# carsonswope/3d-beats

Hardware: AMD Instinct MI355X
Metric: classified Mpix/s on 848x480 depth frames (4 trees, depth 20); % of the bounding roofline level (roofline.bound; HBM: roofline.hbm_frac) (higher is better)
Workload: dtype f32

## Files before the change

3d-beats_amd/csrc/rdf_hip.hip:

```cpp

#include <hip/hip_runtime.h>
#include <stdint.h>
#include <stdio.h>
#include <stdlib.h>
#include <string.h>
#include <time.h>
#include <unistd.h>

#include <algorithm>
#include <array>
#include <atomic>
#include <mutex>
#include <utility>
#include <vector>

#include "../../include/rdf_hip.h"
#include "rdf_device.hpp"
#include "rdf_host_state.hpp"
#include "rdf_launch_plan.hpp"

namespace {

constexpr uint32_t kFlagLeftLeaf = 1u, kFlagRightLeaf = 2u, kFlagExact = 4u;
using rdf_host::kSchedSlots;
// ... 446 lines not shown
                    }
                }
            } else {
                const float *pp = a.forest +
                    ((size_t)tree * (size_t)a.nodes + (leaf >> 1)) * (size_t)a.E +
                    7 + (leaf & 1u) * a.C + c0;
#pragma unroll
                for (int c = 0; c < CMAX; c += 4) {
                    if (c0 + c + 3 < a.C) {
                        const f4u v = *reinterpret_cast<const f4u *>(pp + c);
                        pdf[c] = pdf[c] + v.x; pdf[c + 1] = pdf[c + 1] + v.y;
                        pdf[c + 2] = pdf[c + 2] + v.z; pdf[c + 3] = pdf[c + 3] + v.w;
                    } else {
#pragma unroll
                        for (int e = 0; e < 4; ++e)
                            if (c0 + c + e < a.C) pdf[c + e] = pdf[c + e] + pp[c + e];
                    }
                }
            }
            return true;
        };
        uint32_t tw_h = kIdle, tw_i = 0u;
        bool tw_valid = false;
        for (uint32_t first = TW ? (tw_row < tile_rows ? tw_row * 64u : n_valid) : wave * 64u; first < n_valid; first += BLOCK) {
            const uint32_t slot = first + (uint32_t)lane;
            uint32_t entry = slot;
            bool live = true;
            if (compact) {
                if (slot >= n_valid) {
                    if (!DEEP) continue;
                    live = false;
                }
                entry = px_list[live ? slot : first];
            }
            const int ly = (int)(y0 + (entry >> 6) * fold + ((entry & 63u) >> col_shift));
            const int px = (int)(x0 + (entry & ((1u << col_shift) - 1u)));
            if (!compact && (ly >= a.Hl || px >= a.Wl)) {
                if (!DEEP) continue;
                live = false;
            }
            const uint32_t i = img_loff + (uint32_t)ly * (uint32_t)a.Wl + (uint32_t)px;
            const int x = px * a.r, y = ly * a.r;
            const int xl = x - tx0, yl = y - ty0;
            bool skip = false;
            if (!compact && live && a.filter_class != -1) skip = (int)a.filter[i] != a.filter_class;
            uint32_t d = 0u;
            if (!skip && live) d = (uint32_t)tprobe_value(tprobe_issue(pc, (uint32_t)xl * 2u, (uint32_t)yl));
            if (!compact && live && (skip || d == 0u || d == kNoPixel)) {
                if (a.fill_untouched && (!TW || tw_tree == 0u)) a.labels[i] = (uint16_t)kNoPixel;
                if (!DEEP) continue;
                live = false;
            }
            if (DEEP && !live) d = 1u;
            const float df = (float)d;
            const float r0 = __builtin_amdgcn_rcpf(df);
            const float rcp = __builtin_fmaf(__builtin_fmaf(-df, r0, 1.0f), r0, r0);
            float rcp_s = rcp * (1.0f / kNumScale);
            const float df_s = df * kNumScale;
            uint32_t kx2 = ((uint32_t)xl - kMagicBits) * 2u;
            const uint32_t ky = (uint32_t)yl - kMagicBits;
            pin(kx2);

            float best = 0.0f;
            int best_c = 0;
            bool any_leaf = false;

            for (int c0 = 0; c0 < a.C || c0 == 0; c0 += CMAX) {
                float pdf[CMAX];
#pragma unroll
                for (int c = 0; c < CMAX; ++c) pdf[c] = 0.0f;

                for (int kb = TW ? (int)tw_tree : 0; kb < (TW ? (int)tw_tree + 1 : a.T); kb += GROUP) {
                    uint32_t h[GROUP];
#pragma unroll
                    for (int k = 0; k < GROUP; ++k) h[k] = (live && (kb + k) < a.T) ? 1u : kIdle;

#pragma unroll
                    for (int c = 0; c < CMAX; ++c) pin(pdf[c]);
                    const bool fast_levels = PACKED || K > 0;
                    if (fast_levels) set_round_down(rcp_s);

                    int j = 0;
                    if constexpr (kPlainLevels) {
                        if (a.plain_levels != 0 && kb + GROUP <= a.T && !__any(!live)) {
                            for (; j < walk_levels; ++j) {
                                Node n[GROUP];
                                if (j < K) {
#pragma unroll
                                    for (int k = 0; k < GROUP; ++k) {
                                        const uint32_t tk = (uint32_t)min(kb + k, a.T - 1);
                                        n[k] = decode_node(lds_nodes[tk * lds_pitch + h[k]]);
                                    }
                                } else {
#pragma unroll
                                    for (int k = 0; k < GROUP; ++k) {
                                        const int tk = min(kb + k, a.T - 1);
                                        const char *base = reinterpret_cast<const char *>(a.packed16 + ((size_t)tk << a.D));
                                        n[k] = decode_node(*reinterpret_cast<const uint4 *>(base + h[k] * 16u));
                                    }
                                }
                                uint32_t fl = 0u;
#pragma unroll
                                for (int k = 0; k < GROUP; ++k) fl |= n[k].flags;
                                if (__any((fl & (kFlagLeftLeaf | kFlagRightLeaf | kFlagExact)) != 0u)) break;
                                TileProbe qu[GROUP], qv[GROUP];
#pragma unroll
                                for (int k = 0; k < GROUP; ++k) {
                                    const f2 nu = {n[k].ax, n[k].ay};
                                    const f2 nv = {n[k].bx, n[k].by};
                                    const f2 r2 = {rcp_s, rcp_s};
                                    const f2 m2 = {kMagic, kMagic};
                                    const f2 tu = __builtin_elementwise_fma(nu, r2, m2);
                                    const f2 tv = __builtin_elementwise_fma(nv, r2, m2);
                                    qu[k] = tprobe_issue(pc, (__float_as_uint(tu.x) << 1) + kx2, __float_as_uint(tu.y) + ky);
                                    qv[k] = tprobe_issue(pc, (__float_as_uint(tv.x) << 1) + kx2, __float_as_uint(tv.y) + ky);
                                }
#pragma unroll
                                for (int k = 0; k < GROUP; ++k) {
                                    const int g = tprobe_value(qu[k]) - tprobe_value(qv[k]) - (int)n[k].lo16;
                                    h[k] = walk_step_plain(h[k], g, n[k].w2);
                                }
                            }
                        }
                    }

                    for (; j < walk_levels; ++j) {
                        bool any = false;
#pragma unroll
                        for (int k = 0; k < GROUP; ++k) any |= (int)h[k] > 0;
                        if (!__any(any)) break;

                        const bool in_lds = j < K;
                        float df_e = df;
                        if (!PACKED && fast_levels && j == K) set_round_nearest(df_e);
                        Node n[GROUP];
                        uint32_t hn[GROUP];
#pragma unroll
                        for (int k = 0; k < GROUP; ++k) hn[k] = (uint32_t)max((int)h[k], (PACKED || in_lds) ? 0 : 1 << j);
                        if (in_lds) {
#pragma unroll
                            for (int k = 0; k < GROUP; ++k) {
                                const uint32_t tk = (uint32_t)min(kb + k, a.T - 1);
                                n[k] = decode_node(lds_nodes[tk * lds_pitch + hn[k]]);
                                if (STATS && c0 == 0) st_lds += (int)h[k] > 0 ? 1u : 0u;
                            }
                        } else if (PACKED) {
#pragma unroll
                            for (int k = 0; k < GROUP; ++k) {
                                const int tk = min(kb + k, a.T - 1);
                                const char *base = reinterpret_cast<const char *>(a.packed16 + ((size_t)tk << a.D));
                                n[k] = decode_node(*reinterpret_cast<const uint4 *>(base + hn[k] * 16u));
                                if (STATS && c0 == 0) st_rec += lines_of((int)h[k] > 0, hn[k] * 16u);
                            }
                        } else {
#pragma unroll
                            for (int k = 0; k < GROUP; ++k) {
                                const int tk = min(kb + k, a.T - 1);
                                const float *p = a.forest + ((size_t)tk * (size_t)a.nodes + (hn[k] - 1u)) * (size_t)a.E;
                                if (STATS && c0 == 0) st_rec += lines_of((int)h[k] > 0, (hn[k] - 1u) * (uint32_t)a.E * 4u);
                                const f4u uv = *reinterpret_cast<const f4u *>(p);
                                const f3u tf = *reinterpret_cast<const f3u *>(p + 4);
                                n[k].ax = a.s * uv.x; n[k].ay = a.s * uv.y; n[k].bx = a.s * uv.z; n[k].by = a.s * uv.w;
                                set_threshold(n[k], thresh_to_int(tf.x));
                                n[k].flags = child_flags(tf.y, tf.z) | kFlagExact;
                            }
                        }

                        uint32_t ux[GROUP], uy[GROUP], vx[GROUP], vy[GROUP];
                        uint32_t fl = 0u;
#pragma unroll
                        for (int k = 0; k < GROUP; ++k) fl |= n[k].flags;
                        if (__any((fl & kFlagExact) != 0u)) {
                            const bool switch_mode = PACKED || in_lds;
                            if (switch_mode) set_round_nearest(df_e);
                            if (PACKED || in_lds) {
#pragma unroll
                                for (int k = 0; k < GROUP; ++k) {
                                    if (n[k].flags & kFlagExact) {
                                        const int tk = min(kb + k, a.T - 1);
                                        if (a.forest) {
                                            const float s_exact = (PACKED && a.info) ? a.info->scale : a.s;
                                            const float *p = a.forest +
                                                ((size_t)tk * (size_t)a.nodes + (hn[k] - 1u)) * (size_t)a.E;
                                            n[k].ax = s_exact * p[0]; n[k].ay = s_exact * p[1];
                                            n[k].bx = s_exact * p[2]; n[k].by = s_exact * p[3];
                                        } else {
                                            n[k].ax = n[k].ay = n[k].bx = n[k].by = 0.0f;
                                            if (a.stale_flag) __hip_atomic_store(a.stale_flag, 1u, __ATOMIC_RELAXED, __HIP_MEMORY_SCOPE_SYSTEM);
                                        }
                                    }
                                }
                            }
#pragma unroll
                            for (int k = 0; k < GROUP; ++k) {
                                const float den = (n[k].flags & kFlagExact) ? df_e : df_s;
                                ux[k] = (uint32_t)min(max(add_wrap(xl, floor_i32(n[k].ax / den)), -(1 << 30)), (1 << 30) - 1) * 2u;
                                uy[k] = (uint32_t)add_wrap(yl, floor_i32(n[k].ay / den));
                                vx[k] = (uint32_t)min(max(add_wrap(xl, floor_i32(n[k].bx / den)), -(1 << 30)), (1 << 30) - 1) * 2u;
                                vy[k] = (uint32_t)add_wrap(yl, floor_i32(n[k].by / den));
                            }
                            if (switch_mode) {
#pragma unroll
                                for (int k = 0; k < GROUP; ++k) { pin(ux[k]); pin(uy[k]); pin(vx[k]); pin(vy[k]); }
                                set_round_down(ux[0]);
// ... 274 lines not shown
                int best_c = 0;
                bool any_leaf = false;
                for (int c0 = 0; c0 < a.C || c0 == 0; c0 += CMAX) {
                    float pdf[CMAX];
#pragma unroll
                    for (int c = 0; c < CMAX; ++c) pdf[c] = 0.0f;
                    for (uint32_t t = 0; t < tw_T; ++t)
                        any_leaf |= add_leaf_pdf(xch[(tw_row * tw_T + t) * 64u + (uint32_t)lane], (int)t, c0, pdf);
#pragma unroll
                    for (int c = 0; c < CMAX; ++c) {
                        if (c0 + c < a.C && pdf[c] > best) {
                            best = pdf[c];
                            best_c = c0 + c;
                        }
                    }
                }
                if (a.keep_if_no_leaf && !any_leaf) {
                    if (a.fill_untouched) a.labels[tw_i] = (uint16_t)kNoPixel;
                } else {
                    a.labels[tw_i] = (uint16_t)best_c;
                }
            }
        }
        if (!TW && more_tiles) {
            uint32_t before = 0u;
            if (lane == 0) before = atomicAdd(&s_tile[4u + (it & 1u)], 1u);
            scout = __builtin_amdgcn_readfirstlane((int)before) == 0;
        }
    }

    if (PACKED && a.info && a.stale_flag && block_id == n_blocks - 1u && tid == 0 && !a.q_helper) {
        if (a.info->generation != a.expect_gen)
            __hip_atomic_store(a.stale_flag, 1u, __ATOMIC_RELAXED, __HIP_MEMORY_SCOPE_SYSTEM);
    }

    if (a.sched && queued != 0u && tid == 0) {
        const unsigned int done = atomicAdd(a.sched + 8 * kSchedStride, 1u);
        if (done == q_blocks - 1u) {
            for (int q = 0; q < 9; ++q) atomicExch(a.sched + q * kSchedStride, 0u);
        }
    }

    if (STATS) {
        uint32_t c[8] = {st_px, st_lv, st_lf, st_lds, st_rec, st_leaf, st_far, st_blk};
#pragma unroll
        for (int i = 0; i < 8; ++i) {
            unsigned long long v = c[i];
            for (int o = 32; o > 0; o >>= 1) v += __shfl_down(v, o);
            if (lane == 0 && (i < 3 || a.stats_wide)) atomicAdd(a.stats + i, v);
        }
    }
}

__global__ __launch_bounds__(256) void k_pack(const float *forest, NodeRec16 *packed16, PackInfo *info,
                                              float *packed_pdf, LastLevelRec *last_level, unsigned int *last_level_unusable,
                                              uint4 *deep, int n_trees, int C, int cpad,
                                              size_t total_slots, int D, int E, float s, int force_exact, uint32_t generation)
{
    const size_t slot = (size_t)blockIdx.x * 256 + threadIdx.x;
    if (slot >= total_slots) return;
    const size_t tree = slot >> D, h = slot & (((size_t)1 << D) - 1);
    if (h == 0) {
        NodeRec16 z16 = {{0u, 0u, 0u, 0u}};
        packed16[slot] = z16;
        for (int c = 0; c < 2 * cpad; ++c) packed_pdf[slot * 2 * (size_t)cpad + c] = 0.f;
        if (tree == 0) {
            info->scale = s; info->magic = kPackMagic; info->generation = generation;
            info->n_trees = (uint32_t)n_trees; info->max_depth = (uint32_t)D; info->n_classes = (uint32_t)C;
        }
        if (deep && tree == 0) {
            uint4 *z = deep + (deep_total_lines(n_trees, D, cpad) << 3);
            for (int i = 0; i < 8; ++i) z[i] = make_uint4(0u, 0u, 0u, 0u);
        }
        return;
    }
    const size_t i = tree * ((((size_t)1) << D) - 1) + (h - 1);
    const float *p = forest + i * (size_t)E;
    struct { uint32_t flags; } n;
    NodeRec16 h16 = encode_node(s * p[0], s * p[1], s * p[2], s * p[3], p[4], p[5], p[6]);
    if (force_exact) h16.w[3] |= kFlagExact;
    n.flags = h16.w[3] & 0xFFu;
    packed16[slot] = h16;
    if (n.flags & kFlagExact) atomicAdd(&info->exact_nodes, 1u);
    float *q = packed_pdf + slot * 2 * (size_t)cpad;
    for (int c = 0; c < cpad; ++c) {
        q[c] = c < C ? p[7 + c] : 0.f;
        q[cpad + c] = c < C ? p[7 + C + c] : 0.f;
    }
    if (deep) {
        const int R0 = D - deep_last_levels(cpad), Lmin = R0 % 3;
        const int j = 63 - __clzll((unsigned long long)h);
        if (j >= Lmin) {
            const int R = j >= R0 ? R0 : R0 - 3 * ((R0 - j + 2) / 3);
            const int t = j - R;
            const size_t line = deep_lines_before(n_trees, R, Lmin) + (tree << R) + ((h >> t) - ((size_t)1 << R));
            uint4 *blk = deep + (line << 3);
            const uint4 rec = make_uint4(h16.w[0], h16.w[1], h16.w[2], h16.w[3]);
            const float4 *pq = reinterpret_cast<const float4 *>(q);
            const uint4 z = make_uint4(0u, 0u, 0u, 0u);
            if (R == R0 && cpad == 8) {
                blk[0] = rec; blk[1] = z; blk[6] = z; blk[7] = z;
                for (int i = 0; i < 4; ++i) reinterpret_cast<float4 *>(blk)[2 + i] = pq[i];
            } else {
                blk[((1u << t) - 1u) + (uint32_t)(h & ((1u << t) - 1u))] = rec;
                if (t == 0) blk[7] = z;
                if (R == R0 && t == 1) {
                    const uint32_t c = (uint32_t)(h & 1u);
                    reinterpret_cast<float4 *>(blk)[3 + 2 * c] = pq[0];
                    reinterpret_cast<float4 *>(blk)[4 + 2 * c] = pq[1];
                }
            }
            unsigned int *tr = reinterpret_cast<unsigned int *>(deep + ((deep_total_lines(n_trees, D, cpad) + 1u) << 3));
            if (n.flags & kFlagExact) atomicMax(tr, (unsigned)j + 1u);
            if (j == D - 1 && (n.flags & 7u) != (kFlagLeftLeaf | kFlagRightLeaf)) atomicAdd(tr + 1, 1u);
        }
    }
    const size_t first = (size_t)1 << (D - 1);
    if (last_level && h >= first) {
        LastLevelRec r;
        r.node = h16;
        for (int c = 0; c < 4; ++c) {
            r.pdf_left[c] = q[c];
            r.pdf_right[c] = q[4 + c];
            r.pad[c] = 0u;
        }
        last_level[(tree << (D - 1)) + (h - first)] = r;
        const bool unusable = (n.flags & 7u) != (kFlagLeftLeaf | kFlagRightLeaf);
        const float *pp = forest + (tree * ((((size_t)1) << D) - 1) + ((h >> 1) - 1)) * (size_t)E;
        const float to_me = pp[5 + (h & 1)];
        const bool in_use = to_me >= -1.0f && to_me < 0.0f;
        const unsigned long long bu = __ballot(unusable), bi = __ballot(in_use);
        const unsigned long long mine = __ballot(true);
        if ((unsigned)__lane_id() == (unsigned)__ffsll((long long)mine) - 1u) {
            if (bu) atomicAdd(last_level_unusable, (unsigned)__popcll(bu));
            if (bi) atomicAdd(last_level_unusable + 1, (unsigned)__popcll(bi));
        }
    }
}

constexpr int kMaxSpecLayers = 4;
struct SpecFilters {
    int n;
    int fl[kMaxSpecLayers], fc[kMaxSpecLayers];
};

__global__ __launch_bounds__(256) void k_composite(const uint16_t *const *imgs, int n_images, uint32_t n_px,
                                                   const int2 *cond, int n_cond, uint16_t *out, int32_t *bad,
                                                   int fill_untouched, uint32_t flip_w, const uint32_t *colors,
                                                   int num_colors, uint32_t *rgba, const SpecFilters spec)
{
    const uint32_t p = blockIdx.x * 256u + threadIdx.x;
    if (p >= n_px) return;
    uint32_t lab[kMaxSpecLayers];
    if (spec.n > 0) {
#pragma unroll
        for (int i = 0; i < kMaxSpecLayers; ++i) {
            lab[i] = kNoPixel;
            if (i < spec.n) {
                uint32_t l = imgs[i][p];
                if (spec.fl[i] >= 0) {
                    uint32_t f = kNoPixel;
#pragma unroll
                    for (int j = 0; j < kMaxSpecLayers; ++j)
                        if (j < i && j == spec.fl[i]) f = lab[j];
                    if ((int)f != spec.fc[i] && l != kNoPixel) {
                        l = kNoPixel;
// ... 226 lines not shown
            *split->launched = (int)hgrid;
            return (int)hipGetLastError();
        }
    }
    hipLaunchKernelGGL(kern, dim3((unsigned)grid), dim3(block), lds_bytes, st, ka);
    return (int)hipGetLastError();
}

template <int NL>
int launch_multi(ForestKernel<NL> kern, int block, const EvalArgsN<NL> &ka, int lds_bytes, DeviceState &ds, int cus, hipStream_t st)
{
    int per_cu = 0;
    const int rc = workgroups_per_cu(ds, reinterpret_cast<const void *>(kern), block, lds_bytes, &per_cu);
    if (rc != RDF_OK) return rc;
    long long per_role = (long long)cus * per_cu / NL;
    uint32_t most_tiles = 0;
    for (int l = 0; l < NL; ++l) most_tiles = ka.l[l].n_tiles > most_tiles ? ka.l[l].n_tiles : most_tiles;
    if (per_role > (long long)most_tiles) per_role = most_tiles;
    if (per_role < 1) per_role = 1;
    hipLaunchKernelGGL(kern, dim3((unsigned)(per_role * NL)), dim3(block), lds_bytes, st, ka);
    return (int)hipGetLastError();
}

StaleFlag make_stale_flag()
{
    StaleFlag f;
    void *h = nullptr, *d = nullptr;
    if (hipHostMalloc(&h, 64, hipHostMallocMapped) == hipSuccess && h) {
        memset(h, 0, 64);
        if (hipHostGetDevicePointer(&d, h, 0) == hipSuccess && d) {
            f.host = reinterpret_cast<unsigned int *>(h);
            f.dev = reinterpret_cast<unsigned int *>(d);
        } else {
            (void)hipHostFree(h);
        }
    }
    (void)hipGetLastError();
    return f;
}
bool stale_flag_raised(DeviceState &ds)
{
    if (!ds.take_stale()) return false;
    g_tables.forget_all();
    return true;
}

std::atomic<uint32_t> g_generation{0};
uint32_t next_generation()
{
    uint32_t seed = g_generation.load(std::memory_order_relaxed);
    if (seed == 0u) {
        struct timespec ts;
        clock_gettime(CLOCK_REALTIME, &ts);
        uint32_t s = (uint32_t)ts.tv_nsec * 2654435761u ^ (uint32_t)ts.tv_sec * 40503u ^ ((uint32_t)getpid() << 16);
        s = (s | 1u) & 0x7FFFFFFFu;
        uint32_t expect = 0u;
        g_generation.compare_exchange_strong(expect, s);
    }
    uint32_t g = g_generation.fetch_add(2u, std::memory_order_relaxed) + 2u;
    return g;
}

int packed_info(DeviceState &ds, const void *packed, int n_trees, int max_depth, int n_classes, void *stream, PackedState *out)
{
    if (ds.stale_flag_made() && g_tables.find(packed, out) && out->exact_nodes >= 0) return RDF_OK;
    const void *info_dev = reinterpret_cast<const char *>(packed) + info_offset(n_trees, max_depth, n_classes);
    hipStreamCaptureStatus cap = hipStreamCaptureStatusNone;
    if (stream && hipStreamIsCapturing(reinterpret_cast<hipStream_t>(stream), &cap) == hipSuccess && cap == hipStreamCaptureStatusActive)
        return RDF_ERR_CAPTURE;
    PackInfo host;
    uint32_t trailer[2] = {0u, 0u};
    hipError_t e = hipMemcpyAsync(&host, info_dev, sizeof(host), hipMemcpyDeviceToHost, reinterpret_cast<hipStream_t>(stream));
    const size_t db = deep_bytes(n_trees, max_depth, n_classes);
    if (e == hipSuccess && db != 0)
        e = hipMemcpyAsync(trailer, reinterpret_cast<const char *>(packed) + deep_offset(n_trees, max_depth, n_classes) + db - 128, sizeof(trailer),
                           hipMemcpyDeviceToHost, reinterpret_cast<hipStream_t>(stream));
    if (e == hipSuccess) e = hipStreamSynchronize(reinterpret_cast<hipStream_t>(stream));
    if (e != hipSuccess) return (int)e;
    if (host.magic != kPackMagic || host.generation == 0u || host.n_trees != (uint32_t)n_trees || host.max_depth != (uint32_t)max_depth ||
        host.n_classes != (uint32_t)n_classes)
        return RDF_ERR_BAD_ARG;
    (void)ds.stale_flag(make_stale_flag);
    const uint32_t write_word = g_tables.learn(packed, {host.exact_nodes, host.deep_choice, host.generation, host.scale, info_dev,
                                                        trailer[0], trailer[1]}, out);
    if (write_word != 0u)
        (void)hipMemcpy(reinterpret_cast<char *>(const_cast<void *>(info_dev)) + offsetof(PackInfo, deep_choice), &write_word, sizeof(write_word),
                        hipMemcpyHostToDevice);
    return RDF_OK;
}

int set_deep_choice(const void *packed, int level, bool write_through)
{
    if (!packed) return RDF_ERR_NULL_PTR;
    const void *info_dev = g_tables.set_choice(packed, level);
    if (write_through && info_dev) {
        const uint32_t word = rdf_host::deep_choice_word(level);
        const hipError_t e = hipMemcpy(reinterpret_cast<char *>(const_cast<void *>(info_dev)) + offsetof(PackInfo, deep_choice), &word,
                                       sizeof(word), hipMemcpyHostToDevice);
        if (e != hipSuccess) return (int)e;
    }
    return RDF_OK;
}

int plan_launch(DeviceState *&dsp, const Request &q, Plan *plan)
{
    plan->t_entry = now_ns();
    int rc = check_common(q.depth, q.n_img, q.dim_x, q.dim_y, q.forest ? (const void *)q.forest : q.packed, q.n_trees, q.max_depth,
                          q.n_classes, q.labels_out, q.r);
    if (rc == 1) { plan->empty = true; return RDF_OK; }
    if (rc != 0) return rc;
    if (q.filter_class != -1 && !q.filter) return RDF_ERR_NULL_PTR;
    if (!dsp && (rc = current_device(&dsp)) != 0) return rc;
    DeviceState &ds = *dsp;
    PackedState ps;
    if (q.packed) {
        if (stale_flag_raised(ds)) return RDF_ERR_STALE;
        rc = packed_info(ds, q.packed, q.n_trees, q.max_depth, q.n_classes, q.stream, &ps);
        if (rc != RDF_OK) return rc;
    }
    plan->ds = &ds;
    return plan_shape(q, ps, ds.cus.load(std::memory_order_relaxed), ds.stale_flag_if_made().dev, plan);
}

int dispatch(const Plan &p, void *stream, const SplitSpec *split)
{
    EvalArgs a = p.a;
    DeviceState &ds = *p.ds;
    a.sched = split ? sched_slot(ds, stream, 16 + (split->tag & 3)) : sched_slot(ds, stream);

    hipStream_t st = reinterpret_cast<hipStream_t>(stream);
    const int cus = usable_cus(ds, st);
    const unsigned long long t_launch = now_ns();
    const KernelKey key = select_kernel(p);
    if (key.block == 0) return RDF_ERR_BAD_ARG;
    const ForestKernel<1> kern = forest_kernel<1>(key);
    if (!kern) return RDF_ERR_BUILD;
    if (key.stats && key.packed) a.stats_wide = 1;
    int rc;
    if (key.tw) {
        EvalArgsN<1> ka;
        ka.l[0] = a;
        rc = launch_multi<1>(kern, key.block, ka, p.lds_bytes, ds, cus, st);
    } else {
        rc = launch_one(kern, key.block, a, p.lds_bytes, ds, cus, st, split);
    }
    const unsigned long long t_done = now_ns();
    g_host_ns_plan.fetch_add(t_launch - p.t_entry, std::memory_order_relaxed);
    g_host_ns_launch.fetch_add(t_done - t_launch, std::memory_order_relaxed);
    g_host_calls.fetch_add(1, std::memory_order_relaxed);
    if (rc == RDF_OK) count_kernel_launch(key);
    return rc;
}

int eval_common(const Request &q, const SplitSpec *split = nullptr, DeviceState **dsp = nullptr)
{
    DeviceState *ds = nullptr;
    Plan plan;
    const int rc = plan_launch(dsp ? *dsp : ds, q, &plan);
    return rc != RDF_OK || plan.empty ? rc : dispatch(plan, q.stream, split);
}

template <int NL>
int launch_layers(const Plan *plans, bool tw_all, int cmax, int lds, DeviceState &ds, int cus, hipStream_t st)
{
    EvalArgsN<NL> ka;
    for (int i = 0; i < NL; ++i) ka.l[i] = plans[i].a;
    const KernelKey key = select_layers_kernel(NL, cmax, tw_all);
// ... 615 lines not shown
```

3d-beats_amd/csrc/rdf_host_state.hpp:

```cpp
#pragma once

#include <stdint.h>

#include <atomic>
#include <map>
#include <memory>
#include <mutex>
#include <utility>
#include <vector>

namespace rdf_host {

constexpr int kSchedSlots = 128;
constexpr int kGraphSlots = 384;
constexpr int kMaxDevices = 64;

class SlotPool {
public:
    explicit SlotPool(int limit) : limit_(limit) {}
    int take()
    {
        if (free_.empty()) return next_ < limit_ ? next_++ : -1;
        const int slot = free_.back();
        free_.pop_back();
// ... 59 lines not shown
        std::lock_guard<std::mutex> lock(mu_);
        if (stream_slots) *stream_slots = stream_pool_.in_use();
        if (graph_slots) *graph_slots = graph_pool_.in_use();
    }

    bool occupancy(const void *kernel, int lds_bytes, int *per_cu)
    {
        std::lock_guard<std::mutex> lock(mu_);
        const auto it = occupancy_.find(std::make_pair(kernel, lds_bytes));
        if (it == occupancy_.end()) return false;
        *per_cu = it->second;
        return true;
    }
    void remember_occupancy(const void *kernel, int lds_bytes, int per_cu)
    {
        std::lock_guard<std::mutex> lock(mu_);
        occupancy_[std::make_pair(kernel, lds_bytes)] = per_cu;
    }
    bool usable_cus(const void *stream, int *n)
    {
        std::lock_guard<std::mutex> lock(mu_);
        const auto it = stream_cus_.find(stream);
        if (it == stream_cus_.end()) return false;
        *n = it->second;
        return true;
    }
    void remember_usable_cus(const void *stream, int n)
    {
        std::lock_guard<std::mutex> lock(mu_);
        stream_cus_[stream] = n;
    }

    template <class Alloc>
    StaleFlag stale_flag(Alloc &&alloc)
    {
        std::call_once(stale_once_, [&]() {
            stale_ = alloc();
            stale_made_.store(true, std::memory_order_release);
        });
        return stale_;
    }
    bool stale_flag_made() const { return stale_made_.load(std::memory_order_acquire); }
    StaleFlag stale_flag_if_made() const { return stale_flag_made() ? stale_ : StaleFlag(); }
    bool take_stale()
    {
        unsigned int *const word = stale_flag_if_made().host;
        if (!word || __atomic_load_n(word, __ATOMIC_RELAXED) == 0u) return false;
        return __atomic_exchange_n(word, 0u, __ATOMIC_RELAXED) != 0u;
    }

private:
    std::mutex mu_;
    SlotPool stream_pool_{kSchedSlots}, graph_pool_{kGraphSlots};
    std::map<std::pair<const void *, int>, int> stream_slot_;
    std::map<unsigned long long, std::vector<int>> by_capture_;
    bool graph_exhausted_said_ = false;
    std::map<const void *, int> stream_cus_;
    std::map<std::pair<const void *, int>, int> occupancy_;
    std::once_flag stale_once_;
    std::atomic<bool> stale_made_{false};
    StaleFlag stale_;
};

class DeviceStates {
public:
    DeviceState &at(int ordinal)
    {
        std::call_once(once_[ordinal], [&]() { state_[ordinal].reset(new DeviceState); });
        return *state_[ordinal];
    }

private:
    std::once_flag once_[kMaxDevices];
    std::unique_ptr<DeviceState> state_[kMaxDevices];
};

struct PackedState {
    int deep_from = -1;
    int exact_nodes = -1;
    float scale = 1.0f;
    const void *info_dev = nullptr;
    uint32_t generation = 0;
    uint32_t deep_min_root = 0, deep_bad_last = 0;
};

struct PackedSeen {
    uint32_t exact_nodes, deep_choice, generation;
    float scale;
    const void *info_dev;
    uint32_t deep_min_root, deep_bad_last;
};

inline uint32_t deep_choice_word(int level) { return level < 0 ? 0u : (uint32_t)(level > 30 ? 30 : level) + 1u; }

class PackedTables {
public:
    bool find(const void *table, PackedState *out)
    {
        std::lock_guard<std::mutex> lock(mu_);
        const auto it = known_.find(table);
        if (it == known_.end()) return false;
        *out = it->second;
        return true;
    }
    uint32_t learn(const void *table, const PackedSeen &seen, PackedState *out)
    {
        std::lock_guard<std::mutex> lock(mu_);
        PackedState &st = known_[table];
        st.exact_nodes = (int)(seen.exact_nodes > 0x7FFFFFFFu ? 0x7FFFFFFFu : seen.exact_nodes);
        st.scale = seen.scale;
        st.info_dev = seen.info_dev;
        st.generation = seen.generation;
        st.deep_min_root = seen.deep_min_root;
        st.deep_bad_last = seen.deep_bad_last;
        uint32_t write_word = 0u;
        if (st.deep_from < 0 && seen.deep_choice != 0u && seen.deep_choice <= 31u) st.deep_from = (int)seen.deep_choice - 1;
        else if (st.deep_from >= 0 && seen.deep_choice != (uint32_t)st.deep_from + 1u) write_word = deep_choice_word(st.deep_from);
        *out = st;
        return write_word;
    }
    const void *set_choice(const void *table, int level)
    {
        std::lock_guard<std::mutex> lock(mu_);
        PackedState &st = known_[table];
        st.deep_from = level < 0 ? -1 : level;
        return st.info_dev;
    }
    void forget(const void *table)
    {
        std::lock_guard<std::mutex> lock(mu_);
        known_.erase(table);
    }
    void forget_all()
    {
        std::lock_guard<std::mutex> lock(mu_);
        known_.clear();
    }

private:
    std::mutex mu_;
    std::map<const void *, PackedState> known_;
};

}
```

3d-beats_amd/csrc/rdf_launch_plan.hpp:

```cpp
#pragma once

#include <stdint.h>
#include <stdlib.h>
#include <string.h>

#include <algorithm>
#include <atomic>
#include <mutex>

#include "../../include/rdf_hip.h"
#include "rdf_host_state.hpp"

#ifdef __HIPCC__
#define RDF_HOST_DEVICE __host__ __device__
#else
#define RDF_HOST_DEVICE
#endif

namespace {

constexpr int kGroup = 4;
constexpr int kMaxRowsPerWave = 4;
constexpr int kDefaultLdsBudget = 32700;
constexpr int kDefaultLdsBudget512 = 54600;
constexpr int kDefaultHalo = 32;
constexpr int kMinLdsLevels = 6;

constexpr int kSchedStride = 32;
constexpr int kSchedWords = 9 * kSchedStride;

struct alignas(16) NodeRec16 {
    uint32_t w[4];
};
struct PackInfo {
    uint32_t exact_nodes;
    float scale;
    uint32_t magic;
    uint32_t deep_choice;
    uint32_t generation;
    uint32_t n_trees, max_depth, n_classes;
    uint32_t pad[24];
};
constexpr uint32_t kPackMagic = 0x52444635u;
struct alignas(64) LastLevelRec {
    NodeRec16 node;
    float pdf_left[4], pdf_right[4];
    uint32_t pad[4];
};
static_assert(sizeof(NodeRec16) == 16 && sizeof(PackInfo) == 128 && sizeof(LastLevelRec) == 64, "record sizes");

RDF_HOST_DEVICE inline int deep_last_levels(int cpad) { return cpad == 4 ? 2 : 1; }
RDF_HOST_DEVICE inline size_t deep_lines_before(int n_trees, int R, int Lmin)
{
    return (size_t)n_trees * ((((size_t)1 << R) - ((size_t)1 << Lmin)) / 7u);
}
RDF_HOST_DEVICE inline size_t deep_total_lines(int n_trees, int max_depth, int cpad)
{
    const int R0 = max_depth - deep_last_levels(cpad);
    return deep_lines_before(n_trees, R0, R0 % 3) + ((size_t)n_trees << R0);
}
RDF_HOST_DEVICE inline bool deep_possible(int n_trees, int max_depth, int cpad)
{
    return n_trees >= 1 && (cpad == 4 || cpad == 8) && max_depth >= 5 && max_depth <= 24;
}

#ifdef __HIPCC__
using Vec16 = uint4;
#else
struct alignas(16) Vec16 { uint32_t x, y, z, w; };
#endif

struct EvalArgs {
    const uint16_t *depth;
    const float *forest;
    const NodeRec16 *packed16;
    const uint16_t *filter;
    uint16_t *labels;
    unsigned long long *stats;
    int stats_wide;
    unsigned int *sched;
    uint32_t n_tiles;
    uint32_t tiles_x;
    uint32_t fold;
    uint32_t tiles_y_n;
    int tw_n, th_n, twp_n;
    int halo_xn;
    uint32_t stage_tw8_n, stage_magic_n;
    uint32_t tiles_y;
    int rows_per_wave;
    uint32_t per_img_l;
    uint32_t per_img_d;
    int W, H, Wl, Hl, r;
    int T, D, C, E;
    int nodes;
    int lds_levels;
    int halo;
    int tw, th, twp;
    uint32_t stage_tw8;
    uint32_t stage_magic;
    uint32_t lds_xchg_off;
    uint32_t lds_nodes_off;
    uint32_t lds_mail_off;
    uint32_t lds_list_off;
    uint32_t lds_slab_off;
    const float *packed_pdf;
    const Vec16 *last_level;
    uint32_t last_level_min;
    const Vec16 *deep;
    int deep_from;
    int cpad;
    int filter_class;
    int check_empty;
    int keep_if_no_leaf;
    int fill_untouched;
    int plain_levels;
    float s;
    const PackInfo *info;
    uint32_t expect_gen;
    unsigned int *stale_flag;
    uint32_t q_static, q_blocks;
    int q_helper;
};

template <int NL>
// ... 226 lines not shown
        for (long long pad = 8; !ok_banks && pad <= 64; pad += 8)
            ok_banks = narrow_pitch(s, h, pad, r, fold, vec) && ((s.th_n * s.twp_n * 2 + 15) & ~15ll) <= s.bytes;
        for (long long hx = h - (vec ? 8 : 2); !ok_banks && hx >= 0 && hx >= h - 24; hx -= (vec ? 8 : 2)) {
            ok_banks = narrow_pitch(s, hx, 0, r, fold, vec);
            if (ok_banks) s.hx_n = hx;
        }
        if (!ok_banks) (void)narrow_pitch(s, h, 0, r, fold, vec);
        s.bytes = std::max(s.bytes, (s.th_n * s.twp_n * 2 + 15) & ~15ll);
    }
    return s;
}

int lay_out_lds(const Request &q, const Geometry &g, bool compact_launch, EvalArgs &a)
{
    const int block = g.block, r = q.r, n_trees = q.n_trees, max_depth = q.max_depth;
    const bool coop = g.deep_from_wanted > 0;
    const long long slab_bytes = coop ? (long long)(block / 64) * 8192 : 0;
    const long long budget = coop ? std::min<long long>(coop_lds_budget(block), 163840 - slab_bytes - 2048) : lds_budget(g.tw ? 256 : block);
    const bool many_trees = n_trees >= 8;
    const int halo_default = coop ? (block == 512 ? (many_trees ? 24 : 16) : 8)
                                  : block == 512 ? (r > 1 ? 32 : 56) : (many_trees ? kDefaultHalo + 8 : kDefaultHalo);
    const int halo = g_halo.get(halo_default);
    const int h_min = g.big ? 0 : halo;
    const long long list_bytes = g.tw ? (long long)g.tile_rows * n_trees * 256 :
                                 compact_launch ? (((long long)block * g.rpw * 2 + (long long)g.tile_rows * 4) + 15) & ~15ll : 0;
    int k_forced = g_lds_levels.get(-1);
    if (k_forced > max_depth) k_forced = max_depth;
    while (k_forced > 0 && (long long)n_trees * (1ll << k_forced) * 16 + 32 + list_bytes > budget) --k_forced;
    const int k_min = coop ? (many_trees ? kMinLdsLevels - 2 : kMinLdsLevels - 1)
                           : many_trees ? kMinLdsLevels - 1 : (block == 512 && r == 1 ? kMinLdsLevels + 1 : kMinLdsLevels);
    const int k_floor = k_forced >= 0 ? k_forced : (max_depth < k_min ? max_depth : k_min);
    const long long tile_budget = budget - 32 - list_bytes - (k_floor > 0 ? (long long)n_trees * (1ll << k_floor) * 16 : 0);
    const bool vec_ok = g_stage_vec.get(1) && q.dim_x % 8 == 0 && ((64 * r) % 8 == 0) && (reinterpret_cast<uintptr_t>(q.depth) & 15u) == 0;
    long long tile_bytes = 0;
    for (int h = halo; h >= h_min && h >= 0; h -= 2) {
        const bool vec = vec_ok && h % 8 == 0;
        const TileShape s = tile_shape(h, r, g.tile_rows, a.fold, vec);
        if (s.bytes > tile_budget) continue;
        tile_bytes = s.bytes;
        a.halo = h; a.tw = (int)s.tw; a.th = (int)s.th; a.twp = (int)s.twp;
        a.tw_n = (int)s.tw_n; a.th_n = (int)s.th_n; a.twp_n = (int)s.twp_n; a.halo_xn = (int)s.hx_n;
        if (vec) {
            a.stage_tw8 = (uint32_t)(s.tw >> 3);
            a.stage_magic = (uint32_t)((1ull << 32) / a.stage_tw8) + 1u;
            if (a.fold) {
                a.stage_tw8_n = (uint32_t)(s.tw_n >> 3);
                a.stage_magic_n = (uint32_t)((1ull << 32) / a.stage_tw8_n) + 1u;
            }
        }
        break;
    }
    int K = 0;
    const int k_most = coop ? max_depth - deep_last_levels(a.cpad) : max_depth;
    while (K < k_most && (k_forced < 0 || K < k_forced) &&
           (long long)n_trees * (1ll << (K + 1)) * 16 + tile_bytes + 32 + list_bytes <= budget) ++K;
    a.lds_levels = K;
    bool llt_by_setter = false;
    const int want_llt = g_last_level_table.get(1, &llt_by_setter);
    if (q.packed && want_llt != 0 && !g.tw && max_depth - 1 >= K && last_level_bytes(n_trees, max_depth, q.n_classes) != 0) {
        a.last_level = reinterpret_cast<const Vec16 *>(reinterpret_cast<const char *>(a.packed_pdf) +
                                                       ((size_t)n_trees << max_depth) * 2 * (size_t)a.cpad * sizeof(float));
        const int pct = llt_by_setter && want_llt == 1 ? 0 : g_env_last_level_min_pct.get(50);
        a.last_level_min = (uint32_t)((((unsigned long long)n_trees << (max_depth - 1)) * (unsigned long long)(pct < 0 ? 0 : pct > 100 ? 100 : pct)) / 100u);
    }
    if (coop) {
        const int R0 = max_depth - deep_last_levels(a.cpad);
        int from = g.deep_from_wanted;
        if (from < K) from = K;
        if (from > R0) from = R0;
        from = R0 - 3 * ((R0 - from) / 3);
        a.deep = reinterpret_cast<const Vec16 *>(reinterpret_cast<const char *>(q.packed) + deep_offset(n_trees, max_depth, q.n_classes));
        a.deep_from = from;
    }
    const long long node_bytes = K > 0 ? (long long)n_trees * (1ll << K) * 16 : 0;
    a.lds_nodes_off = (uint32_t)tile_bytes;
    a.lds_mail_off = (uint32_t)(tile_bytes + node_bytes);
    a.lds_list_off = (uint32_t)(tile_bytes + node_bytes + 32);
    a.lds_xchg_off = a.lds_list_off;
    const long long slab_at = (tile_bytes + node_bytes + 32 + list_bytes + 1023) & ~1023ll;
    a.lds_slab_off = (uint32_t)slab_at;
    return coop ? (int)(slab_at + slab_bytes) : (int)(node_bytes + tile_bytes + 32 + list_bytes);
}

int plan_shape(const Request &q, const PackedState &ps, int device_cus, unsigned int *stale_flag_dev, Plan *plan)
{
    EvalArgs &a = plan->a;
    memset(&a, 0, sizeof(a));
    a.depth = q.depth; a.forest = q.forest; a.filter = q.filter; a.labels = q.labels_out;
    a.stats = q.stats;
    a.W = q.dim_x; a.H = q.dim_y; a.Wl = q.dim_x / q.r; a.Hl = q.dim_y / q.r; a.r = q.r;
    a.per_img_l = (uint32_t)a.Wl * (uint32_t)a.Hl;
    a.per_img_d = (uint32_t)q.dim_x * (uint32_t)q.dim_y;
    a.T = q.n_trees; a.D = q.max_depth; a.C = q.n_classes; a.E = 7 + 2 * q.n_classes;
    a.nodes = (int)((1ll << q.max_depth) - 1);
    a.filter_class = q.filter_class;
    a.keep_if_no_leaf = q.keep_if_no_leaf;
    a.fill_untouched = q.fill_untouched;
    a.s = q.s;
    if (q.packed) {
        const size_t slots = (size_t)q.n_trees << q.max_depth;
        a.packed16 = reinterpret_cast<const NodeRec16 *>(q.packed);
        a.packed_pdf = reinterpret_cast<const float *>(a.packed16 + slots);
        a.cpad = classes_padded(q.n_classes);
        if (ps.exact_nodes > 0 && !q.forest) return RDF_ERR_NULL_PTR;
        a.s = ps.scale;
        a.info = reinterpret_cast<const PackInfo *>(ps.info_dev);
        a.expect_gen = ps.generation;
        a.stale_flag = stale_flag_dev;
    }
    const bool compaction = g_compaction.get(1) != 0;
    const Geometry &g = plan->g = choose_geometry(q, a.Wl, a.Hl, device_cus, ps, compaction);
    if (g.n_tiles >= (1ll << 31)) return RDF_ERR_TOO_LARGE;
    a.fold = g.fold; a.tiles_x = g.tiles_x; a.tiles_y = g.tiles_y; a.tiles_y_n = g.tiles_y_n;
    a.n_tiles = (uint32_t)g.n_tiles; a.rows_per_wave = g.rpw;
    a.plain_levels = g_plain_levels.get(1) != 0;
    a.check_empty = (g.big || q.r > 1) ? 1 : g_env_check_empty_small.get(0);
    plan->compact_launch = q.packed && !q.stats && q.filter_class != -1 && compaction;
    plan->lds_bytes = lay_out_lds(q, g, plan->compact_launch, a);
    plan->deep = g.deep_from_wanted > 0;
    plan->packed = q.packed != nullptr; plan->stats = q.stats != nullptr;
    return RDF_OK;
}

struct KernelKey {
    int block; bool packed; int cmax; bool stats; int group; bool compact; int nl; bool tw; bool deep;
};
constexpr bool operator==(const KernelKey &a, const KernelKey &b)
{
    return a.block == b.block && a.packed == b.packed && a.cmax == b.cmax && a.stats == b.stats && a.group == b.group &&
           a.compact == b.compact && a.nl == b.nl && a.tw == b.tw && a.deep == b.deep;
}

constexpr KernelKey kForestKernels[] = {
    {256, true, 4, false, 1, false, 1, false, false},  {512, true, 4, false, 1, false, 1, false, false},
    {256, true, 4, false, 2, false, 1, false, false},  {512, true, 4, false, 2, false, 1, false, false},
    {256, true, 4, false, 3, false, 1, false, false},  {512, true, 4, false, 3, false, 1, false, false},
    {256, true, 4, false, 4, false, 1, false, false},  {512, true, 4, false, 4, false, 1, false, false},
    {256, true, 8, false, 1, false, 1, false, false},  {512, true, 8, false, 1, false, 1, false, false},
    {256, true, 8, false, 2, false, 1, false, false},  {512, true, 8, false, 2, false, 1, false, false},
    {256, true, 8, false, 3, false, 1, false, false},  {512, true, 8, false, 3, false, 1, false, false},
    {256, true, 8, false, 4, false, 1, false, false},  {512, true, 8, false, 4, false, 1, false, false},
    {256, true, 16, false, 1, false, 1, false, false}, {512, true, 16, false, 1, false, 1, false, false},
    {256, true, 16, false, 4, false, 1, false, false}, {512, true, 16, false, 4, false, 1, false, false},
    {256, true, 4, false, 4, true, 1, false, false},   {512, true, 4, false, 4, true, 1, false, false},
    {256, true, 8, false, 4, true, 1, false, false},   {512, true, 8, false, 4, true, 1, false, false},
    {256, true, 16, false, 4, true, 1, false, false},  {512, true, 16, false, 4, true, 1, false, false},
    {256, false, 4, false, 1, false, 1, false, false},  {512, false, 4, false, 1, false, 1, false, false},
    {256, false, 4, false, 4, false, 1, false, false},  {512, false, 4, false, 4, false, 1, false, false},
    {256, false, 16, false, 1, false, 1, false, false}, {512, false, 16, false, 1, false, 1, false, false},
    {256, false, 16, false, 4, false, 1, false, false}, {512, false, 16, false, 4, false, 1, false, false},
    {256, false, 4, true, 4, false, 1, false, false},
    {256, true, 4, true, 4, false, 1, false, false},   {512, true, 4, true, 4, false, 1, false, false},
    {256, true, 4, true, 4, false, 1, false, true},    {512, true, 4, true, 4, false, 1, false, true},
    {256, true, 4, false, 2, false, 1, false, true},   {512, true, 4, false, 2, false, 1, false, true},
    {256, true, 4, false, 3, false, 1, false, true},   {512, true, 4, false, 3, false, 1, false, true},
    {256, true, 4, false, 4, false, 1, false, true},   {512, true, 4, false, 4, false, 1, false, true},
    {256, true, 4, false, 4, true, 1, false, true},    {512, true, 4, false, 4, true, 1, false, true},
    {256, true, 8, false, 2, false, 1, false, true},   {512, true, 8, false, 2, false, 1, false, true},
    {256, true, 8, false, 3, false, 1, false, true},   {512, true, 8, false, 3, false, 1, false, true},
    {256, true, 8, false, 4, false, 1, false, true},   {512, true, 8, false, 4, false, 1, false, true},
    {256, true, 8, false, 4, true, 1, false, true},    {512, true, 8, false, 4, true, 1, false, true},
    {512, true, 4, false, 1, false, 1, true, false},   {512, true, 8, false, 1, false, 1, true, false},
    {512, true, 4, false, 1, false, 2, true, false},   {512, true, 8, false, 1, false, 2, true, false},
    {512, true, 4, false, 1, false, 3, true, false},   {512, true, 8, false, 1, false, 3, true, false},
    {256, true, 4, false, 4, false, 2, false, false},  {256, true, 8, false, 4, false, 2, false, false},
    {256, true, 4, false, 4, false, 3, false, false},  {256, true, 8, false, 4, false, 3, false, false},
};
constexpr int kNumForestKernels = (int)(sizeof(kForestKernels) / sizeof(kForestKernels[0]));

inline int kernel_index(const KernelKey &key)
{
    for (int i = 0; i < kNumForestKernels; ++i)
        if (kForestKernels[i] == key) return i;
    return -1;
}

KernelKey select_kernel(const Plan &p)
{
    const EvalArgs &a = p.a;
    const int block = p.g.block == 512 ? 512 : 256;
    if (p.g.tw) return {512, true, a.C <= 4 ? 4 : 8, false, 1, false, 1, true, false};
    if (p.stats && p.packed) {
        if (a.C > 4 || p.compact_launch) return {};
        return {block, true, 4, true, 4, false, 1, false, p.deep};
    }
    if (p.stats) return {256, false, 4, true, 4, false, 1, false, false};
    const int g = group_for(a, p.packed);
    if (p.deep) {
        const int cmax = a.cpad == 4 ? 4 : 8;
        if (p.compact_launch) return {block, true, cmax, false, 4, true, 1, false, true};
        return {block, true, cmax, false, g <= 2 ? 2 : g == 3 ? 3 : 4, false, 1, false, true};
    }
    if (!p.packed) return {block, false, a.C <= 4 ? 4 : 16, false, g, false, 1, false, false};
    const int cmax = a.C <= 4 ? 4 : a.C <= 8 ? 8 : 16;
    if (p.compact_launch) return {block, true, cmax, false, 4, true, 1, false, false};
    return {block, true, cmax, false, g == 1 ? 1 : (g == 2 || g == 3) && cmax <= 8 ? g : 4, false, 1, false, false};
}

// ... 7 lines not shown
```

Measured before the change: 14550.

## Precompute leaf-free prefix depth at pack time to drop per-level leaf checks

During forest packing, each node that is a leaf or exact node records its level in a census via atomicMax. This fixes how many top levels are guaranteed free of leaves and exact nodes across the whole forest. The plain walk loop then runs exactly that many levels, with no per-level flag OR and no __any vote/break. LDS and global-memory levels are split into separate loops. This removes a wave-wide reduction and a branch from every level, but needs an extra PackInfo field, one host readback of it, and an atomic in the pack kernel.

```diff
diff --git a/3d-beats_amd/csrc/rdf_hip.hip b/3d-beats_amd/csrc/rdf_hip.hip
--- a/3d-beats_amd/csrc/rdf_hip.hip
+++ b/3d-beats_amd/csrc/rdf_hip.hip
@@ -552,30 +552,14 @@
 
                     int j = 0;
                     if constexpr (kPlainLevels) {
-                        if (a.plain_levels != 0 && kb + GROUP <= a.T && !__any(!live)) {
-                            for (; j < walk_levels; ++j) {
+                        if (kb + GROUP <= a.T && !__any(!live)) {
+                            const int plain_n = min(walk_levels, a.plain_levels);
+                            auto plain_level = [&](const uint4 (&w)[GROUP]) __attribute__((always_inline)) {
                                 Node n[GROUP];
-                                if (j < K) {
-#pragma unroll
-                                    for (int k = 0; k < GROUP; ++k) {
-                                        const uint32_t tk = (uint32_t)min(kb + k, a.T - 1);
-                                        n[k] = decode_node(lds_nodes[tk * lds_pitch + h[k]]);
-                                    }
-                                } else {
-#pragma unroll
-                                    for (int k = 0; k < GROUP; ++k) {
-                                        const int tk = min(kb + k, a.T - 1);
-                                        const char *base = reinterpret_cast<const char *>(a.packed16 + ((size_t)tk << a.D));
-                                        n[k] = decode_node(*reinterpret_cast<const uint4 *>(base + h[k] * 16u));
-                                    }
-                                }
-                                uint32_t fl = 0u;
-#pragma unroll
-                                for (int k = 0; k < GROUP; ++k) fl |= n[k].flags;
-                                if (__any((fl & (kFlagLeftLeaf | kFlagRightLeaf | kFlagExact)) != 0u)) break;
                                 TileProbe qu[GROUP], qv[GROUP];
 #pragma unroll
                                 for (int k = 0; k < GROUP; ++k) {
+                                    n[k] = decode_node(w[k]);
                                     const f2 nu = {n[k].ax, n[k].ay};
                                     const f2 nv = {n[k].bx, n[k].by};
                                     const f2 r2 = {rcp_s, rcp_s};
@@ -590,6 +574,25 @@
                                     const int g = tprobe_value(qu[k]) - tprobe_value(qv[k]) - (int)n[k].lo16;
                                     h[k] = walk_step_plain(h[k], g, n[k].w2);
                                 }
+                            };
+                            for (const int lds_n = min(plain_n, K); j < lds_n; ++j) {
+                                uint4 w[GROUP];
+#pragma unroll
+                                for (int k = 0; k < GROUP; ++k) {
+                                    const uint32_t tk = (uint32_t)min(kb + k, a.T - 1);
+                                    w[k] = lds_nodes[tk * lds_pitch + h[k]];
+                                }
+                                plain_level(w);
+                            }
+                            for (; j < plain_n; ++j) {
+                                uint4 w[GROUP];
+#pragma unroll
+                                for (int k = 0; k < GROUP; ++k) {
+                                    const int tk = min(kb + k, a.T - 1);
+                                    const char *base = reinterpret_cast<const char *>(a.packed16 + ((size_t)tk << a.D));
+                                    w[k] = *reinterpret_cast<const uint4 *>(base + h[k] * 16u);
+                                }
+                                plain_level(w);
                             }
                         }
                     }
@@ -1030,6 +1033,10 @@
     n.flags = h16.w[3] & 0xFFu;
     packed16[slot] = h16;
     if (n.flags & kFlagExact) atomicAdd(&info->exact_nodes, 1u);
+    if (n.flags & (kFlagLeftLeaf | kFlagRightLeaf | kFlagExact)) {
+        const unsigned int v = (unsigned int)(D - (63 - __clzll((unsigned long long)h)));
+        if (__hip_atomic_load(&info->plain_census, __ATOMIC_RELAXED, __HIP_MEMORY_SCOPE_AGENT) < v) atomicMax(&info->plain_census, v);
+    }
     float *q = packed_pdf + slot * 2 * (size_t)cpad;
     for (int c = 0; c < cpad; ++c) {
         q[c] = c < C ? p[7 + c] : 0.f;
@@ -1422,7 +1429,7 @@
         return RDF_ERR_BAD_ARG;
     (void)ds.stale_flag(make_stale_flag);
     const uint32_t write_word = g_tables.learn(packed, {host.exact_nodes, host.deep_choice, host.generation, host.scale, info_dev,
-                                                        trailer[0], trailer[1]}, out);
+                                                        trailer[0], trailer[1], host.plain_census}, out);
     if (write_word != 0u)
         (void)hipMemcpy(reinterpret_cast<char *>(const_cast<void *>(info_dev)) + offsetof(PackInfo, deep_choice), &write_word, sizeof(write_word),
                         hipMemcpyHostToDevice);
diff --git a/3d-beats_amd/csrc/rdf_host_state.hpp b/3d-beats_amd/csrc/rdf_host_state.hpp
--- a/3d-beats_amd/csrc/rdf_host_state.hpp
+++ b/3d-beats_amd/csrc/rdf_host_state.hpp
@@ -165,6 +165,7 @@
     const void *info_dev = nullptr;
     uint32_t generation = 0;
     uint32_t deep_min_root = 0, deep_bad_last = 0;
+    uint32_t plain_census = 0;
 };
 
 struct PackedSeen {
@@ -172,6 +173,7 @@
     float scale;
     const void *info_dev;
     uint32_t deep_min_root, deep_bad_last;
+    uint32_t plain_census;
 };
 
 inline uint32_t deep_choice_word(int level) { return level < 0 ? 0u : (uint32_t)(level > 30 ? 30 : level) + 1u; }
@@ -196,6 +198,7 @@
         st.generation = seen.generation;
         st.deep_min_root = seen.deep_min_root;
         st.deep_bad_last = seen.deep_bad_last;
+        st.plain_census = seen.plain_census;
         uint32_t write_word = 0u;
         if (st.deep_from < 0 && seen.deep_choice != 0u && seen.deep_choice <= 31u) st.deep_from = (int)seen.deep_choice - 1;
         else if (st.deep_from >= 0 && seen.deep_choice != (uint32_t)st.deep_from + 1u) write_word = deep_choice_word(st.deep_from);
diff --git a/3d-beats_amd/csrc/rdf_launch_plan.hpp b/3d-beats_amd/csrc/rdf_launch_plan.hpp
--- a/3d-beats_amd/csrc/rdf_launch_plan.hpp
+++ b/3d-beats_amd/csrc/rdf_launch_plan.hpp
@@ -39,7 +39,8 @@
     uint32_t deep_choice;
     uint32_t generation;
     uint32_t n_trees, max_depth, n_classes;
-    uint32_t pad[24];
+    uint32_t plain_census;
+    uint32_t pad[23];
 };
 constexpr uint32_t kPackMagic = 0x52444635u;
 struct alignas(64) LastLevelRec {
@@ -432,6 +433,12 @@
     return coop ? (int)(slab_at + slab_bytes) : (int)(node_bytes + tile_bytes + 32 + list_bytes);
 }
 
+inline int plain_levels_of(uint32_t census, int max_depth, int knob)
+{
+    if (knob == 0 || census == 0u || max_depth < 1 || census > (uint32_t)max_depth) return 0;
+    return max_depth - (int)census;
+}
+
 int plan_shape(const Request &q, const PackedState &ps, int device_cus, unsigned int *stale_flag_dev, Plan *plan)
 {
     EvalArgs &a = plan->a;
@@ -463,7 +470,7 @@
     if (g.n_tiles >= (1ll << 31)) return RDF_ERR_TOO_LARGE;
     a.fold = g.fold; a.tiles_x = g.tiles_x; a.tiles_y = g.tiles_y; a.tiles_y_n = g.tiles_y_n;
     a.n_tiles = (uint32_t)g.n_tiles; a.rows_per_wave = g.rpw;
-    a.plain_levels = g_plain_levels.get(1) != 0;
+    a.plain_levels = q.packed ? plain_levels_of(ps.plain_census, q.max_depth, g_plain_levels.get(1)) : 0;
     a.check_empty = (g.big || q.r > 1) ? 1 : g_env_check_empty_small.get(0);
     plan->compact_launch = q.packed && !q.stats && q.filter_class != -1 && compaction;
     plan->lds_bytes = lay_out_lds(q, g, plan->compact_launch, a);
```

Result: no change. 14640 (median of 6 runs) (+0.6%).
